# mdangschat/ctc-asr

Hardware: AMD Instinct MI355X
Metric: audio-seconds/s training throughput (DS2, 10 s utterances) (higher is better)
Workload: dtype f32 tensors / accumulate / own kernels; projection GEMMs: fp16x3 split (22 significand bits) where the layer input is bounded or, behind a ReLU cell, scaled per row / per column on the device - forward projections and their gradient GEMMs - bf16x6 split (24 bits) elsewhere; forward and backward recu

## Files before the change

ctc_asr_amd/csrc/wgrad16.hip:

```cpp
#include "common.h"

namespace {

typedef _Float16 f16x8 __attribute__((ext_vector_type(8)));
typedef unsigned int u32x4 __attribute__((ext_vector_type(4)));
union WgFrag {
    u32x4 u;
    f16x8 h;
};

constexpr int WG_THREADS = 512;
constexpr int WG_TILE = 256;
constexpr int WG_A_BYTES = (WG_TILE / 16) * 2 * 1024, WG_B_BYTES = WG_A_BYTES;
constexpr int WG_STAGE_BYTES = WG_A_BYTES + WG_B_BYTES;
constexpr size_t WG_LDS_BYTES = 2 * (size_t)WG_STAGE_BYTES;
constexpr int WG_LOADERS = 4;

struct WgArgs {
    const char *a;
    const char *b[2];
    float *out[2];
    int64_t ld[2];
    const float *inv;
    float alpha[2];
    int m, n[2], stage0[2];
    int stages, m_tiles, n_tiles[2], tiles_n[2], tiles_m;
    int parts;
    int *sync;
    long spin_limit;
};

long g_wgrad_spin_limit = 1L << 24;

__device__ __forceinline__ void wg_dma16(const char *base, unsigned lane_off, unsigned lds_base) {
    unsigned keep;
    asm volatile("s_mov_b32 %0, m0\n\ts_mov_b32 m0, %3\n\ts_nop 0\n\t"
                 "global_load_lds_dwordx4 %1, %2\n\ts_mov_b32 m0, %0"
                 : "=&s"(keep)
                 : "v"(lane_off), "s"(base), "s"(lds_base)
                 : "memory");
}

__global__ void __launch_bounds__(WG_THREADS) wgrad16_kernel(WgArgs p) {
    extern __shared__ __attribute__((aligned(16))) char smem[];
    __shared__ int gave_up;
    const int tid = threadIdx.x, lane = tid & 63;
    const int wave = __builtin_amdgcn_readfirstlane(tid >> 6);
    const int wr = wave >> 2, wc = wave & 3;
    if (p.parts > 1 &&
        __hip_atomic_load(p.sync, __ATOMIC_RELAXED, __HIP_MEMORY_SCOPE_AGENT) != 0)
        return;
    if (tid == 0) gave_up = 0;
    const int tiles_all = p.tiles_m * (p.tiles_n[0] + p.tiles_n[1]);
    const int part = blockIdx.x / tiles_all, tile_id = blockIdx.x % tiles_all;
    const int s_lo = (int)((int64_t)p.stages * part / p.parts);
    const int s_hi = (int)((int64_t)p.stages * (part + 1) / p.parts);
    int v = tile_id, which = 0;
    if (v >= p.tiles_m * p.tiles_n[0]) {
        v -= p.tiles_m * p.tiles_n[0];
        which = 1;
    }
    int tm, tn;
    {
        const int tiles_n = p.tiles_n[which], count = p.tiles_m * tiles_n;
        if (p.tiles_m % 4 == 0 && tiles_n % 4 == 0 && count % 8 == 0 &&
            (p.tiles_m * p.tiles_n[0]) % 8 == 0) {
            const int pos = (v % 8) * (count / 8) + v / 8;
            const int block = pos / 16, in_block = pos % 16, blocks_n = tiles_n / 4;
            tm = (block / blocks_n) * 4 + in_block / 4;
            tn = (block % blocks_n) * 4 + in_block % 4;
        } else {
            tm = v / tiles_n;
            tn = v % tiles_n;
        }
    }
    const int nt_total = p.n_tiles[which];
    const int mt0 = tm * (WG_TILE / 16), nt0 = tn * (WG_TILE / 16);
    const char *b_all = p.b[which] + (size_t)p.stage0[which] * nt_total * 2048;
    const unsigned lds0 = __builtin_amdgcn_readfirstlane(
        (unsigned)(uintptr_t)(__attribute__((address_space(3))) char *)smem);
    const unsigned lane16 = lane * 16;
    unsigned a_chunk[8], b_chunk[8];
#pragma unroll
    for (int c = 0; c < 8; ++c) {
        const int chunk = (wave % WG_LOADERS) * 8 + c;
        a_chunk[c] = __builtin_amdgcn_readfirstlane(
            (unsigned)(min(mt0 + (chunk >> 1), p.m_tiles - 1) * 2048 + (chunk & 1) * 1024));
        b_chunk[c] = __builtin_amdgcn_readfirstlane(
            (unsigned)(min(nt0 + (chunk >> 1), nt_total - 1) * 2048 + (chunk & 1) * 1024));
    }
    auto issue = [&](int s, unsigned buf) {
        if (wave >= WG_LOADERS) return;
        const char *a_base = p.a + (size_t)s * p.m_tiles * 2048;
        const char *b_base = b_all + (size_t)s * nt_total * 2048;
#pragma unroll
        for (int c = 0; c < 8; ++c) {
            wg_dma16(b_base + b_chunk[c], lane16, buf + WG_A_BYTES + (wave * 8 + c) * 1024);
            wg_dma16(a_base + a_chunk[c], lane16, buf + (wave * 8 + c) * 1024);
        }
    };

    f32x4 total[8][4];
#pragma unroll
    for (int i = 0; i < 8; ++i)
#pragma unroll
        for (int j = 0; j < 4; ++j) total[i][j] = (f32x4){0.f, 0.f, 0.f, 0.f};

    issue(s_lo, lds0);
    for (int s = s_lo; s < s_hi; ++s) {
        const int par = (s - s_lo) & 1;
        const char *cur = smem + par * WG_STAGE_BYTES;
        asm volatile("s_waitcnt vmcnt(0)" ::: "memory");
        __syncthreads();
        if (s + 1 < s_hi) issue(s + 1, lds0 + (par ^ 1) * WG_STAGE_BYTES);
        const char *a_rd = cur + wr * (8 * 2048) + lane * 16;
        const char *b_rd = cur + WG_A_BYTES + wc * (4 * 2048) + lane * 16;
        WgFrag x1[4], x2[4];
#pragma unroll
        for (int j = 0; j < 4; ++j) {
            x1[j].u = *reinterpret_cast<const u32x4 *>(b_rd + j * 2048);
            x2[j].u = *reinterpret_cast<const u32x4 *>(b_rd + j * 2048 + 1024);
        }
#pragma unroll
        for (int i = 0; i < 8; ++i) {
            WgFrag d1, d2;
            d1.u = *reinterpret_cast<const u32x4 *>(a_rd + i * 2048);
            d2.u = *reinterpret_cast<const u32x4 *>(a_rd + i * 2048 + 1024);
#pragma unroll
            for (int j = 0; j < 4; ++j)
                total[i][j] = __builtin_amdgcn_mfma_f32_16x16x32_f16(d1.h, x1[j].h, total[i][j], 0, 0, 0);
#pragma unroll
            for (int j = 0; j < 4; ++j)
                total[i][j] = __builtin_amdgcn_mfma_f32_16x16x32_f16(d1.h, x2[j].h, total[i][j], 0, 0, 0);
#pragma unroll
            for (int j = 0; j < 4; ++j)
                total[i][j] = __builtin_amdgcn_mfma_f32_16x16x32_f16(d2.h, x1[j].h, total[i][j], 0, 0, 0);
        }
    }

    float *out = p.out[which];
    const int64_t ld = p.ld[which];
    const float alpha = p.alpha[which];
    const int n_cols = p.n[which];
    if (p.parts == 1) {
#pragma unroll
        for (int i = 0; i < 8; ++i) {
#pragma unroll
            for (int r = 0; r < 4; ++r) {
                const int m = (mt0 + 8 * wr + i) * 16 + 4 * (lane >> 4) + r;
                if (m >= p.m) continue;
                const float scale = p.inv[m] * alpha;
                float *row = out + (int64_t)m * ld;
#pragma unroll
                for (int j = 0; j < 4; ++j) {
                    const int n = (nt0 + 4 * wc + j) * 16 + (lane & 15);
                    if (n < n_cols) row[n] += total[i][j][r] * scale;
                }
            }
        }
// ... 40 lines not shown
                const int n = (nt0 + 4 * wc + j) * 16 + (lane & 15);
                if (n < n_cols)
                    __hip_atomic_store(row + n, have[r][j] + total[i][j][r] * scale,
                                       __ATOMIC_RELAXED, __HIP_MEMORY_SCOPE_AGENT);
            }
        }
    }
    asm volatile("s_waitcnt vmcnt(0)" ::: "memory");
    __syncthreads();
    if (tid == 0)
        __hip_atomic_store(turn, part + 1 == p.parts ? 0 : part + 1, __ATOMIC_RELAXED,
                           __HIP_MEMORY_SCOPE_AGENT);
}

__global__ void __launch_bounds__(256) wgrad16_pack_kernel(const float *x, int64_t ld,
                                                           int64_t rows_total, int cols,
                                                           int64_t row0, const float *col_scale,
                                                           float scale, char *out, int col_tiles) {
    const int stage = blockIdx.x;
    const int c = blockIdx.y * 64 + (threadIdx.x & 63), kg = threadIdx.x >> 6;
    if (c >= col_tiles * 16) return;
    const float cs = (c < cols ? (col_scale ? col_scale[c] : 1.f) : 0.f) * scale;
    const int64_t r = row0 + (int64_t)stage * 32 + 8 * kg;
    unsigned pc[8];
#pragma unroll
    for (int e = 0; e < 8; ++e) {
        const int64_t row = r + e;
        float v = (c < cols && row >= 0 && row < rows_total) ? x[row * ld + c] * cs : 0.f;
        v = fminf(fmaxf(v, -60000.f), 60000.f);
        const _Float16 h1 = (_Float16)v;
        const _Float16 h2 = (_Float16)(v - (float)h1);
        pc[e] = (unsigned)__builtin_bit_cast(unsigned short, h1) |
                ((unsigned)__builtin_bit_cast(unsigned short, h2) << 16);
    }
    const u32x4 first = {(pc[0] & 0xFFFFu) | (pc[1] << 16), (pc[2] & 0xFFFFu) | (pc[3] << 16),
                         (pc[4] & 0xFFFFu) | (pc[5] << 16), (pc[6] & 0xFFFFu) | (pc[7] << 16)};
    const u32x4 second = {(pc[0] >> 16) | (pc[1] & 0xFFFF0000u), (pc[2] >> 16) | (pc[3] & 0xFFFF0000u),
                          (pc[4] >> 16) | (pc[5] & 0xFFFF0000u), (pc[6] >> 16) | (pc[7] & 0xFFFF0000u)};
    char *dst = out + (((size_t)stage * col_tiles + (c >> 4)) * 2) * 1024 + (kg * 16 + (c & 15)) * 16;
    *reinterpret_cast<u32x4 *>(dst) = first;
    *reinterpret_cast<u32x4 *>(dst + 1024) = second;
}

}

void wgrad16_set_spin_limit(long polls) { g_wgrad_spin_limit = polls > 0 ? polls : 1L << 24; }

extern "C" size_t ctcasr_wgrad16_packed_bytes(int stages, int cols) {
    return stages > 0 && cols > 0 ? (size_t)stages * ((cols + 15) / 16) * 2048 : 0;
}

extern "C" size_t ctcasr_wgrad16_sync_ints(int m, int nx, int ny) {
    const int tm = (m + WG_TILE - 1) / WG_TILE;
    return 1 + (size_t)tm * ((nx + WG_TILE - 1) / WG_TILE + (ny > 0 ? (ny + WG_TILE - 1) / WG_TILE : 0));
}

extern "C" int ctcasr_wgrad16_pack(const float *x, int64_t ld_x, int64_t rows_total, int cols,
                                   int64_t row0, int stages, const float *col_scale, float scale,
                                   void *packed, ctcasr_stream_t stream) {
    if (!x || !packed || rows_total <= 0 || cols <= 0 || ld_x < cols || stages <= 0 ||
        !(scale > 0.f))
        return CTCASR_ERR_BAD_ARGUMENT;
    const int col_tiles = (cols + 15) / 16;
    wgrad16_pack_kernel<<<dim3(stages, (col_tiles * 16 + 63) / 64), 256, 0, (hipStream_t)stream>>>(
        x, ld_x, rows_total, cols, row0, col_scale, scale, reinterpret_cast<char *>(packed),
        col_tiles);
    return ctcasr_launch_status();
}

extern "C" int ctcasr_wgrad16_gemm(const void *d_packed, int m, int stages, const float *inv_scale,
                                   const void *x_packed, int x_stage0, int nx, float x_scale,
                                   float *dw_x, int64_t ld_x, const void *y_packed, int y_stage0,
                                   int ny, float y_scale, float *dw_y, int64_t ld_y,
                                   int parts, int32_t *sync, ctcasr_stream_t stream) {
    if (!d_packed || !inv_scale || !x_packed || !dw_x || m <= 0 || stages <= 0 || nx <= 0 ||
        ld_x < nx || x_stage0 < 0 || !(x_scale > 0.f) ||
        parts < 1 || parts > stages || (parts > 1 && !sync) ||
        (y_packed && (!dw_y || ny <= 0 || ld_y < ny || y_stage0 < 0 || !(y_scale > 0.f))))
        return CTCASR_ERR_BAD_ARGUMENT;
    static bool attr_set = false;
    if (!attr_set) {
        if (hipFuncSetAttribute(reinterpret_cast<const void *>(wgrad16_kernel),
                                hipFuncAttributeMaxDynamicSharedMemorySize,
                                (int)WG_LDS_BYTES) != hipSuccess)
            return CTCASR_ERR_LAUNCH;
        attr_set = true;
    }
    WgArgs a = {};
    a.a = reinterpret_cast<const char *>(d_packed);
    a.m = m; a.stages = stages; a.inv = inv_scale;
    a.m_tiles = (m + 15) / 16;
    a.tiles_m = (m + WG_TILE - 1) / WG_TILE;
    a.b[0] = reinterpret_cast<const char *>(x_packed); a.stage0[0] = x_stage0; a.n[0] = nx;
    a.alpha[0] = 1.0f / x_scale; a.out[0] = dw_x; a.ld[0] = ld_x;
    a.n_tiles[0] = (nx + 15) / 16; a.tiles_n[0] = (nx + WG_TILE - 1) / WG_TILE;
    if (y_packed) {
        a.b[1] = reinterpret_cast<const char *>(y_packed); a.stage0[1] = y_stage0; a.n[1] = ny;
        a.alpha[1] = 1.0f / y_scale; a.out[1] = dw_y; a.ld[1] = ld_y;
        a.n_tiles[1] = (ny + 15) / 16; a.tiles_n[1] = (ny + WG_TILE - 1) / WG_TILE;
    }
    a.parts = parts; a.sync = sync; a.spin_limit = g_wgrad_spin_limit;
    const int tiles = a.tiles_m * (a.tiles_n[0] + a.tiles_n[1]) * parts;
    wgrad16_kernel<<<tiles, WG_THREADS, WG_LDS_BYTES, (hipStream_t)stream>>>(a);
    return ctcasr_launch_status();
}
```

ctc_asr_amd/hip.py:

```python

import ctypes
import functools
import os

import torch

_PKG_DIR = os.path.dirname(os.path.abspath(__file__))
LIB_PATH = os.path.join(_PKG_DIR, 'libctcasr.so')

ABI_VERSION = 7
BUILD_PROBE_WRONG_RESULTS, BUILD_NONDEFAULT_TUNING = 1, 2
RNN_DEFAULT, RNN_HALF_CHIP, RNN_WHOLE_CHIP, RNN_ONE_BARRIER = 0, 1, 2, 4
RNN_REDUCE_SCATTER = 8
RNN_F16 = 16
RNN_XCD_SPLIT = 32
RNN_STAGGER = 64
RNN_KPAIR = 128
CELL_IDS = {'rnn_relu': 0, 'rnn_tanh': 1, 'lstm': 2, 'gru': 3}
CELL_GATES = {'rnn_relu': 1, 'rnn_tanh': 1, 'lstm': 4, 'gru': 3}

_c_int, _c_i64, _c_u64 = ctypes.c_int, ctypes.c_int64, ctypes.c_uint64
_c_f, _c_p, _c_sz = ctypes.c_float, ctypes.c_void_p, ctypes.c_size_t

SIGNATURES = {
# ... 66 lines not shown
                                   _c_p]),
    'ctcasr_split_f16': (_c_int, [_c_p, _c_i64, _c_int, _c_i64, _c_f, _c_p, _c_int, _c_p, _c_i64,
                                  _c_i64, _c_p]),
    'ctcasr_colmax_scale': (_c_int, [_c_p, _c_i64, _c_int, _c_i64, _c_p, _c_p, _c_p, _c_p]),
    'ctcasr_colscale_from_max': (_c_int, [_c_p, _c_int, _c_p, _c_p, _c_p]),
    'ctcasr_split_f16_cols': (_c_int, [_c_p, _c_i64, _c_int, _c_i64, _c_p, _c_f, _c_p, _c_int, _c_p,
                                       _c_i64, _c_i64, _c_p]),
    'ctcasr_split_f16_rows': (_c_int, [_c_p, _c_i64, _c_int, _c_i64, _c_p, _c_int, _c_p, _c_i64,
                                       _c_i64, _c_p, _c_p]),
    'ctcasr_rescale_rows': (_c_int, [_c_p, _c_i64, _c_p, _c_f, _c_p, _c_i64, _c_i64, _c_int, _c_int,
                                     _c_p]),
    'ctcasr_gemm_split_nt': (_c_int, [_c_p, _c_i64, _c_p, _c_i64, _c_p, _c_i64, _c_int, _c_int, _c_int,
                                      _c_int, _c_p]),
    'ctcasr_gemm_split_tn': (_c_int, [_c_p, _c_i64, _c_p, _c_i64, _c_p, _c_i64, _c_int, _c_int, _c_int,
                                      _c_int, _c_p]),
    'ctcasr_rnn_f16_recurrence': (_c_int, [_c_int] * 7),
    'ctcasr_collective_traffic': (_c_int, [_c_int, _c_int, _c_p, _c_p, _c_i64, _c_i64, _c_p]),
    'ctcasr_wgrad16_packed_bytes': (_c_sz, [_c_int, _c_int]),
    'ctcasr_wgrad16_pack': (_c_int, [_c_p, _c_i64, _c_i64, _c_int, _c_i64, _c_int, _c_p, _c_f, _c_p,
                                     _c_p]),
    'ctcasr_wgrad16_gemm': (_c_int, [_c_p, _c_int, _c_int, _c_p, _c_p, _c_int, _c_int, _c_f, _c_p,
                                     _c_i64, _c_p, _c_int, _c_int, _c_f, _c_p, _c_i64, _c_int, _c_p,
                                     _c_p]),
    'ctcasr_wgrad16_sync_ints': (_c_sz, [_c_int, _c_int, _c_int]),
    'ctcasr_dgrad16_packed_bytes': (_c_sz, [_c_int]),
    'ctcasr_dgrad16_pack_weights': (_c_int, [_c_p, _c_i64, _c_int, _c_int, _c_f, _c_p, _c_p]),
    'ctcasr_dgrad16_supported': (_c_int, [_c_int] * 4),
    'ctcasr_dgrad16_published_offsets': (_c_int, [_c_int, _c_int, _c_int, _c_p, _c_p]),
    'ctcasr_dgrad16_blockscaled': (_c_int, [_c_p, _c_int, _c_int, _c_int, _c_p, _c_f, _c_int, _c_p,
                                            _c_i64] + [_c_int] * 5 + [_c_p]),
    'ctcasr_features_num_frames': (_c_int, [_c_int]),
    'ctcasr_features_tables_bytes': (_c_sz, []),
    'ctcasr_features_init_tables': (_c_int, [_c_p, _c_int, _c_p]),
    'ctcasr_features_workspace_bytes': (_c_sz, [_c_int, _c_int]),
    'ctcasr_features': (_c_int, [_c_p, _c_p] + [_c_int] * 5 + [_c_p, _c_p, _c_int, _c_p, _c_p,
                                 _c_sz, _c_p]),
    'ctcasr_adam_step': (_c_int, [_c_p] * 4 + [_c_i64] + [_c_f] * 4 + [_c_i64, _c_f, _c_p, _c_p]),
    'ctcasr_step_guard': (_c_int, [_c_p, _c_p, _c_int, _c_p, _c_p, _c_p, _c_p, _c_p]),
    'ctcasr_rnn_timeout_word_offset': (_c_sz, [_c_int] * 5),
    'ctcasr_absmax': (_c_int, [_c_p, _c_i64, _c_p, _c_p]),
    'ctcasr_occupy_cus': (_c_int, [_c_int, _c_int, _c_p]),
}

_lib = None

EVENTS = None
# ... 643 lines not shown

@_on_tensor_device
def wgrad16_pack(x, rows_total, row0, stages, scale, col_scale=None, out=None):
    if x.dim() != 2 or x.dtype != torch.float32 or not x.is_cuda or x.stride(1) != 1:
        raise CtcAsrError('wgrad16_pack: x must be an f32 matrix in HBM with unit column stride.')
    cols = x.shape[1]
    need = load().ctcasr_wgrad16_packed_bytes(int(stages), cols)
    if out is None:
        out = torch.empty(need, dtype=torch.uint8, device=x.device)
    elif out.dtype != torch.uint8 or out.numel() < need or not out.is_contiguous():
        raise CtcAsrError('wgrad16_pack: out must be a contiguous uint8 buffer of {} bytes.'
                          .format(need))
    _check(load().ctcasr_wgrad16_pack(
        x.data_ptr(), x.stride(0), int(rows_total), cols, int(row0), int(stages),
        _dev(col_scale, name='col_scale'), float(scale), out.data_ptr(), _stream()),
        'wgrad16_pack')
    return out


@_on_tensor_device
def wgrad16_gemm(d_packed, m, stages, inv_scale, x_packed, x_stage0, x_scale, dw_x,
                 y_packed=None, y_stage0=0, y_scale=1.0, dw_y=None, parts=1):
    parts = max(1, min(int(parts), int(stages)))
    sync = None
    if parts > 1:
        need = load().ctcasr_wgrad16_sync_ints(int(m), dw_x.shape[1], 0 if dw_y is None else dw_y.shape[1])
        sync = _WGRAD16_SYNC.get(dw_x.device.index)
        if sync is None or sync.numel() < need:
            sync = _WGRAD16_SYNC[dw_x.device.index] = torch.zeros(max(need, 4096), dtype=torch.int32,
                                                            device=dw_x.device)
    for name, t in (('dw_x', dw_x), ('dw_y', dw_y)):
        if t is not None and (t.dim() != 2 or t.dtype != torch.float32 or not t.is_cuda or
                              t.stride(1) != 1 or t.shape[0] != m):
            raise CtcAsrError('wgrad16_gemm: {} must be an f32 [m, n] view in HBM with unit '
                              'column stride.'.format(name))
    _check(load().ctcasr_wgrad16_gemm(
        d_packed.data_ptr(), int(m), int(stages), _dev(inv_scale, name='inv_scale'),
        x_packed.data_ptr(), int(x_stage0), dw_x.shape[1], float(x_scale), dw_x.data_ptr(),
        dw_x.stride(0), None if y_packed is None else y_packed.data_ptr(), int(y_stage0),
        0 if dw_y is None else dw_y.shape[1], float(y_scale),
        None if dw_y is None else dw_y.data_ptr(), 0 if dw_y is None else dw_y.stride(0),
        parts, None if sync is None else sync.data_ptr(), _stream()), 'wgrad16_gemm')


_WGRAD16_SYNC = {}


def _wgrad16_sync_of(device):
    device = torch.device(device)
    return _WGRAD16_SYNC.get(torch.cuda.current_device() if device.index is None else device.index)


def wgrad16_gave_up_waiting(device):
    sync = _wgrad16_sync_of(device)
    return bool(sync is not None and int(sync[0].item()) != 0)


def wgrad16_check(device):
    sync = _wgrad16_sync_of(device)
    if sync is not None and int(sync[0].item()) != 0:
        sync.zero_()
        torch.cuda.synchronize(sync.device)
        raise CtcAsrError('wgrad16_gemm: a part of a weight-gradient tile timed out waiting for '
                          'its turn to add; the step\'s update was not applied ({}).'.format(
                              load().ctcasr_error_string(-5).decode()))



# ... 422 lines not shown
```

ctc_asr_amd/model.py:

```python

import math
import os

import numpy as np
import torch

from ctc_asr_amd import hip, metrics, split_gemm
from ctc_asr_amd.labels import num_classes

CONV_KERNEL_SIZES = ((11, 41), (11, 21), (11, 21))
CONV_STRIDES = ((2, 2), (1, 2), (1, 2))
GATES = {'lstm': 4, 'gru': 3, 'rnn_relu': 1, 'rnn_tanh': 1}


class InfeasibleAlignmentError(ValueError):
    """Raised where ``tf.nn.ctc_loss`` raises InvalidArgumentError ("Not enough time for target
    transition sequence"), ``ignore_longer_outputs_than_inputs=False`` (``asr/model.py:259``)."""


class ModelConfig:

    def __init__(self, used_model='ds2', conv_filters=(32, 32, 96), num_units_dense=2048,
                 num_layers_rnn=4, num_units_rnn=2048, rnn_cell='rnn_relu', cudnn=True,
                 relu_cutoff=20.0, conv_dropout_rate=0.0, rnn_dropout_rate=0.0,
# ... 296 lines not shown
        self.arena = ParamArena(cfg, self.device)
        self.arena.load(params if params is not None else init_params(cfg, seed))
        self.step_count = 0
        self.overlap_wgrad = os.environ.get('CTCASR_OVERLAP_WGRAD', '1') == '1'
        self.own_conv = os.environ.get('CTCASR_OWN_CONV', '1') == '1'
        self._conv_packed = {}
        self._conv_packed16 = {}
        self.conv_f16 = os.environ.get('CTCASR_CONV_F16', '1') == '1'
        self.conv_wrw_f16 = os.environ.get('CTCASR_CONV_WRW_F16', '1') == '1'
        self.conv_fused_bwd = os.environ.get('CTCASR_CONV_FUSED_BWD', '1') == '1'
        self.side_gate_max_us = int(os.environ.get('CTCASR_SIDE_GATE_US', '300'))
        self._ticket = 0
        self.bwd_chunks = max(0, int(os.environ.get('CTCASR_BWD_CHUNKS', '0')))
        self.fwd_chunks = max(1, int(os.environ.get('CTCASR_FWD_CHUNKS', '4')))
        self.fwd_pipeline_max_batch = int(os.environ.get('CTCASR_FWD_PIPELINE_MAX_BATCH', '16'))
        self.split_gemm = os.environ.get('CTCASR_SPLIT_GEMM', '1') == '1'
        self.split_dense4 = os.environ.get('CTCASR_SPLIT_DENSE4', '1') == '1'
        self.fwd_f16 = os.environ.get('CTCASR_FWD_F16', '1') == '1'
        self.bwd_f16 = os.environ.get('CTCASR_BWD_F16', '1') == '1'
        self.split_wgrad = os.environ.get('CTCASR_SPLIT_WGRAD', '1') == '1'
        self.own_dgrad = os.environ.get('CTCASR_OWN_DGRAD', '1') == '1'
        self.own_wgrad = os.environ.get('CTCASR_OWN_WGRAD', '1') == '1'
        self.own_wgrad_parts = int(os.environ.get('CTCASR_WGRAD_PARTS', '2'))
        self.unbounded_f16 = os.environ.get('CTCASR_UNBOUNDED_F16', '1') == '1'
        self.dgrad_early = os.environ.get('CTCASR_DGRAD_EARLY', '0')
        self._dgrad_stream = None
        self.rnn_fwd_f16 = os.environ.get('CTCASR_RNN_FWD_F16', '1') == '1'
        self.rnn_bwd_f16 = os.environ.get('CTCASR_RNN_BWD_F16', '1') == '1'
        self.rnn_xcd_flag = hip.RNN_XCD_SPLIT \
            if os.environ.get('CTCASR_RNN_XCD_SPLIT', '1') == '1' else 0
        self.rnn_stagger_flag = hip.RNN_STAGGER \
            if os.environ.get('CTCASR_RNN_STAGGER', '1') == '1' else 0
        if os.environ.get('CTCASR_RNN_KPAIR', '0') == '1':
            self.rnn_stagger_flag |= hip.RNN_KPAIR
        self.rnn_kpair_wide = os.environ.get('CTCASR_RNN_KPAIR_2048', '1') == '1'
        self.rnn_fwd_pieces = os.environ.get('CTCASR_RNN_FWD_PIECES', '1') == '1'
        self._w_split, self._w_split_ready, self._w_split_bufs = {}, None, {}
        self._w_guard = None
        self._side_stream = None
        self.early_hooks = False
        self.rnn_bwd_flags = int(os.environ.get('CTCASR_RNN_BWD_FLAGS', str(hip.RNN_DEFAULT)))
        self.gpu_metrics = os.environ.get('CTCASR_GPU_METRICS', '1') == '1'
        self._rnn_ws = {}
        self.dropout_seed = int(seed) * 0x9E3779B1 + 1
        self._acts = None
        self._w_hh_t = [torch.empty((2, cfg.num_units_rnn, GATES[cfg.cell] * cfg.num_units_rnn),
# ... 644 lines not shown
                g['dense4/kernel'].zero_()
                split_gemm.wgrad16(g['dense4/kernel'], pieces.buf, inv,
                                   split_gemm.Split(dz16, split_gemm.H_B), scale, 0,
                                   x_col_inv=dz_inv)
            elif k4_split is not None:
                if dz_split is None:
                    dz_split = split_gemm.split(dz, split_gemm.B_ORDER)
                if acts['flat_split'] is None:
                    acts['flat_split'] = split_gemm.split(acts['rnn_flat'], split_gemm.A_ORDER)
                split_gemm.mm_tn_rows(g['dense4/kernel'], acts['flat_split'], dz_split, 0, rows,
                                      accumulate=False)
            else:
                torch.mm(acts['rnn_flat'].t(), dz, out=g['dense4/kernel'])
            if early:
                done('dense4')

        on_side([dz] + ([dz_split.buf] if dz_split is not None else []) +
                ([acts['flat_split'].buf] if acts['flat_split'] is not None else []),
                dense4_weight_grad, gate=True)
        if not early:
            deferred.append('dense4')

        need_dx_first = True
        rnn_rate = acts['rnn_rate']
        for i in range(cfg.num_layers_rnn - 1, -1, -1):
            name = 'rnn{}'.format(i)
            x, y = acts['layer_in'][i], acts['layer_out'][i]
            seeds = acts['drop_seeds'][i]
            if seeds[1] is not None:
                dy = hip.dropout(dy.contiguous(), rnn_rate, seeds[1])
            gh = gates * hidden
            chunks = 1
            if (side is not main and acts['rnn_len'] is None and not whole_chip_rnn and
                    persistent):
                chunks = self.bwd_chunks or 2
                if t_out < 8 * chunks:
                    chunks = 1
            dy = dy.contiguous()
            dxw = torch.empty((t_out, batch, 2, gh), dtype=torch.float32, device=dy.device)

            drec = hip.rnn_gru_drec(acts['reserves'][i], t_out, batch, hidden) if cell == 'gru' \
                else dxw
            dxw2d = dxw.view(rows, 2 * gh)
            w_ih = p[name + '/w_ih'].view(2 * gh, -1)

            w_pieces = self._weight_split(name, True, acts)
# ... 32 lines not shown

            side_tensors = [dxw] + [t.buf for t in (ds, drs, acts['in_split'][i],
                                                    acts['flat_split']) if t is not None] + \
                [t[0].buf for t in (x16, y16)
                 if t is not None and not isinstance(t, split_gemm.ColScaled)]

            def split_steps(lo, hi, ds=ds, drs=drs, dxw2d=dxw2d, drec=drec):
                for d, (a, b) in enumerate(((lo, hi), (t_out - hi, t_out - lo))):
                    rng, cols = slice(a * batch, b * batch), slice(d * gh, (d + 1) * gh)
                    hip.split_bf16(dxw2d[rng, cols], split_gemm.B_ORDER, out=ds.buf[rng, :, cols])
                    if drs is not ds:
                        hip.split_bf16(drec.view(rows, 2 * gh)[rng, cols], split_gemm.B_ORDER,
                                       out=drs.buf[rng, :, cols])

            x_packs = {}

            def partial_weight_grads_f16(lo, hi, name=name, dxw2d=dxw2d, drec=drec, x16=x16,
                                         y16=y16, x=x, y=y, colmax=None, x_packs=x_packs):
                own = (self.own_wgrad and cell != 'gru' and
                       not isinstance(x16, split_gemm.ColScaled) and
                       not isinstance(y16, split_gemm.ColScaled))
                for d, (a, b) in enumerate(((lo, hi), (t_out - hi, t_out - lo))):
                    cols = slice(d * gh, (d + 1) * gh)
                    if own:
                        n_rows = (b - a) * batch
                        stages = (n_rows + 31) // 32
                        d_rows = dxw2d[a * batch:b * batch, cols]
                        scale, inv = hip.colmax_scale(d_rows) if colmax is None else \
                            hip.colscale_from_max(colmax[d * gh:(d + 1) * gh])
                        d_pk = hip.wgrad16_pack(d_rows, n_rows, 0, stages, 1.0, col_scale=scale)
                        x_pk = x_packs.pop((a, n_rows), None)
                        if x_pk is None:
                            x_pk = hip.wgrad16_pack(x.view(rows, -1), rows, a * batch, stages,
                                                    x16[1])
                            x_packs[(a, n_rows)] = x_pk
                        y_pk = hip.wgrad16_pack(
                            y.view(rows, 2 * hidden)[:, d * hidden:(d + 1) * hidden], rows,
                            (a + (1 if d else -1)) * batch, stages, y16[1])
                        hip.wgrad16_gemm(d_pk, gh, stages, inv, x_pk, 0, x16[1],
                                         g[name + '/w_ih'][d], y_packed=y_pk, y_scale=y16[1],
                                         dw_y=g[name + '/w_hh'][d], parts=self.own_wgrad_parts)
                        continue
                    d16, inv = split_gemm.wgrad16_operand(
                        dxw2d[a * batch:b * batch, cols],
                        None if colmax is None else colmax[d * gh:(d + 1) * gh])
                    split_gemm.wgrad16(g[name + '/w_ih'][d], d16, inv, x16[0], x16[1], a * batch,
# ... 157 lines not shown
                             colmax=None if colmax is None else colmax[chunks - 1]):
                if cell != 'gru':
                    g[name + '/b_hh'].copy_(g[name + '/b_ih'])
                if chunks > 1 or use_split:
                    partial_weight_grads(0, last, colmax=colmax)
                    return
                torch.mm(dxw2d.t(), x.view(rows, -1),
                         out=g[name + '/w_ih'].view(2 * gates * hidden, -1))
                if t_out > 1:
                    gh = gates * hidden
                    torch.mm(drec[1:, :, 0, :].reshape((t_out - 1) * batch, gh).t(),
                             y[:-1, :, :hidden].reshape((t_out - 1) * batch, hidden),
                             out=g[name + '/w_hh'][0])
                    torch.mm(drec[:-1, :, 1, :].reshape((t_out - 1) * batch, gh).t(),
                             y[1:, :, hidden:].reshape((t_out - 1) * batch, hidden),
                             out=g[name + '/w_hh'][1])

            def layer_weight_grads(name=name, weight_grads=weight_grads):
                weight_grads()
                if early:
                    done(name)

            on_side(side_tensors, layer_weight_grads, gate=i > 0, beside_recurrence=i > 0)
            if not early:
                deferred.append(name)
            if dy_below is not None:
                dy = dy_below
        with torch.cuda.stream(side):
            for name in deferred:
                done(name)
            if hasattr(reduce_hook, 'flush'):
                reduce_hook.flush()

        if cfg.used_model == 'ds2':
            conv_out = acts['conv_out']
            last = conv_out[-1]
            if acts['last_time_major']:
                dact = dy.contiguous().view(last.shape)
            else:
                b_, c_, tt, ff = last.shape
                dact = dy.view(tt, b_, ff, c_).permute(1, 0, 2, 3).contiguous()
            if side is not main and any(kind is None for kind in acts['conv_own']):
                main.wait_stream(side)
            for i in range(len(cfg.conv_filters) - 1, -1, -1):
                name = 'conv{}'.format(i)
                tm = acts['last_time_major'] and i == len(cfg.conv_filters) - 1
# ... 201 lines not shown
```

include/ctcasr.h:

```cpp
#ifndef CTCASR_H_
#define CTCASR_H_

#include <stddef.h>
#include <stdint.h>

#ifdef __cplusplus
extern "C" {
#endif

#define CTCASR_ABI_VERSION 7

enum {
    CTCASR_OK = 0,
    CTCASR_ERR_BAD_ARGUMENT = -1,
    CTCASR_ERR_UNSUPPORTED = -2,
    CTCASR_ERR_WORKSPACE = -3,
    CTCASR_ERR_LAUNCH = -4,
    CTCASR_ERR_TIMEOUT = -5
};

enum {
    CTCASR_CELL_RNN_RELU = 0,
    CTCASR_CELL_RNN_TANH = 1,
    CTCASR_CELL_LSTM = 2,
// ... 174 lines not shown
int ctcasr_gemm_split_tn(const float *a, int64_t lda, const float *b, int64_t ldb, float *c,
                         int64_t ldc, int m, int n, int k, int accumulate, ctcasr_stream_t stream);

size_t ctcasr_dgrad16_packed_bytes(int n);
int ctcasr_dgrad16_published_offsets(int T, int B, int hidden, size_t *exchange,
                                     size_t *inverse_scales);
int ctcasr_dgrad16_pack_weights(const float *w_ih, int64_t ld_w, int hidden, int n, float scale,
                                void *packed, ctcasr_stream_t stream);
int ctcasr_dgrad16_supported(int cell, int T, int B, int hidden);
int ctcasr_dgrad16_blockscaled(void *workspace, int T, int B, int hidden, const void *packed,
                               float scale, int n, float *dx, int64_t ld_dx, int t_lo, int t_hi,
                               int dir_lo, int dir_hi, int accumulate, ctcasr_stream_t stream);

size_t ctcasr_wgrad16_packed_bytes(int stages, int cols);
size_t ctcasr_wgrad16_sync_ints(int m, int nx, int ny);
int ctcasr_wgrad16_pack(const float *x, int64_t ld_x, int64_t rows_total, int cols, int64_t row0,
                        int stages, const float *col_scale, float scale, void *packed,
                        ctcasr_stream_t stream);
int ctcasr_wgrad16_gemm(const void *d_packed, int m, int stages, const float *inv_scale,
                        const void *x_packed, int x_stage0, int nx, float x_scale, float *dw_x,
                        int64_t ld_x, const void *y_packed, int y_stage0, int ny, float y_scale,
                        float *dw_y, int64_t ld_y, int parts, int32_t *sync, ctcasr_stream_t stream);

int ctcasr_adam_step(float *param, const float *grad, float *m, float *v, int64_t n, float lr,
                     float beta1, float beta2, float epsilon, int64_t step, float grad_scale,
                     const int32_t *skip, ctcasr_stream_t stream);
int ctcasr_step_guard(const int32_t *ctc_status, const float *per_utterance_loss, int batch,
                      const uint32_t *timeout_word0, const uint32_t *timeout_word1,
                      const int32_t *wgrad_word, int32_t *skip, ctcasr_stream_t stream);
size_t ctcasr_rnn_timeout_word_offset(int cell, int T, int B, int H, int block);
int ctcasr_occupy_cus(int workgroups, int busy_us, ctcasr_stream_t stream);
int ctcasr_collective_traffic(int workgroups, int busy_us, float *a, const float *b,
                              int64_t scratch_floats, int64_t payload_bytes,
                              ctcasr_stream_t stream);
int ctcasr_absmax(const float *x, int64_t n, uint32_t *max_bits, ctcasr_stream_t stream);

int ctcasr_features_num_frames(int num_samples);
size_t ctcasr_features_tables_bytes(void);
int ctcasr_features_init_tables(void *tables, int sampling_rate, ctcasr_stream_t stream);
size_t ctcasr_features_workspace_bytes(int B, int max_samples);
int ctcasr_features(const int16_t *pcm, const int32_t *num_samples, int B, int max_samples,
                    int feature_type, int normalization, int drop_every_second_frame,
                    const void *tables, float *out, int out_frames, int32_t *out_len,
                    void *workspace, size_t workspace_bytes, ctcasr_stream_t stream);

#ifdef __cplusplus
// ... 4 lines not shown
```

Baseline: 6697.

## Fuse gradient packing into wgrad GEMM and share whole-layer operand packs

Adds an in-place wgrad16 kernel variant that reads the f32 gradient directly, scales it per column, splits it into fp16 hi/lo pairs and writes them to LDS inside the GEMM main loop. This removes the separate pack kernel and the packed round trip through HBM for the A operand. The model also packs each layer's x and y activations once for the whole sequence and reuses those packs across both directions, addressing them by stage and tile offsets. The cost is strided f32 global loads and split arithmetic inside the GEMM loop, more register pressure, and packs kept alive across directions.

Result: no change. 6727, median of 6 (+0.4%).

```diff
diff --git a/ctc_asr_amd/csrc/wgrad16.hip b/ctc_asr_amd/csrc/wgrad16.hip
--- a/ctc_asr_amd/csrc/wgrad16.hip
+++ b/ctc_asr_amd/csrc/wgrad16.hip
@@ -18,7 +18,12 @@
 
 struct WgArgs {
     const char *a;
+    const float *a32;
+    const float *a_scale;
+    int64_t a_ld;
+    int a_rows;
     const char *b[2];
+    int b_tiles[2], b_tile0[2];
     float *out[2];
     int64_t ld[2];
     const float *inv;
@@ -41,6 +46,24 @@
                  : "memory");
 }
 
+__device__ __forceinline__ void wg_split8(const float (&x)[8], u32x4 &first, u32x4 &second) {
+    unsigned pc[8];
+#pragma unroll
+    for (int e = 0; e < 8; ++e) {
+        float v = x[e];
+        v = fminf(fmaxf(v, -60000.f), 60000.f);
+        const _Float16 h1 = (_Float16)v;
+        const _Float16 h2 = (_Float16)(v - (float)h1);
+        pc[e] = (unsigned)__builtin_bit_cast(unsigned short, h1) |
+                ((unsigned)__builtin_bit_cast(unsigned short, h2) << 16);
+    }
+    first = (u32x4){(pc[0] & 0xFFFFu) | (pc[1] << 16), (pc[2] & 0xFFFFu) | (pc[3] << 16),
+                    (pc[4] & 0xFFFFu) | (pc[5] << 16), (pc[6] & 0xFFFFu) | (pc[7] << 16)};
+    second = (u32x4){(pc[0] >> 16) | (pc[1] & 0xFFFF0000u), (pc[2] >> 16) | (pc[3] & 0xFFFF0000u),
+                     (pc[4] >> 16) | (pc[5] & 0xFFFF0000u), (pc[6] >> 16) | (pc[7] & 0xFFFF0000u)};
+}
+
+template <bool INPLACE>
 __global__ void __launch_bounds__(WG_THREADS) wgrad16_kernel(WgArgs p) {
     extern __shared__ __attribute__((aligned(16))) char smem[];
     __shared__ int gave_up;
@@ -76,7 +99,8 @@
     }
     const int nt_total = p.n_tiles[which];
     const int mt0 = tm * (WG_TILE / 16), nt0 = tn * (WG_TILE / 16);
-    const char *b_all = p.b[which] + (size_t)p.stage0[which] * nt_total * 2048;
+    const int b_tiles = p.b_tiles[which];
+    const char *b_all = p.b[which] + ((size_t)p.stage0[which] * b_tiles + p.b_tile0[which]) * 2048;
     const unsigned lds0 = __builtin_amdgcn_readfirstlane(
         (unsigned)(uintptr_t)(__attribute__((address_space(3))) char *)smem);
     const unsigned lane16 = lane * 16;
@@ -92,13 +116,47 @@
     auto issue = [&](int s, unsigned buf) {
         if (wave >= WG_LOADERS) return;
         const char *a_base = p.a + (size_t)s * p.m_tiles * 2048;
-        const char *b_base = b_all + (size_t)s * nt_total * 2048;
+        const char *b_base = b_all + (size_t)s * b_tiles * 2048;
 #pragma unroll
         for (int c = 0; c < 8; ++c) {
             wg_dma16(b_base + b_chunk[c], lane16, buf + WG_A_BYTES + (wave * 8 + c) * 1024);
-            wg_dma16(a_base + a_chunk[c], lane16, buf + (wave * 8 + c) * 1024);
+            if (!INPLACE) wg_dma16(a_base + a_chunk[c], lane16, buf + (wave * 8 + c) * 1024);
         }
     };
+    const int a_c = tid & 255, a_kg = tid >> 8;
+    const int a_col = INPLACE ? min(mt0 * 16 + a_c, p.m - 1) : 0;
+    const float a_cs = INPLACE ? p.a_scale[a_col] : 0.f;
+    const float *a_src = INPLACE ? p.a32 + a_col : nullptr;
+    const unsigned a_dst = (a_c >> 4) * 2048 + (a_kg * 16 + (a_c & 15)) * 16;
+    float a_val[2][8];
+    auto load_a = [&](int s) {
+        const float *src = a_src + (int64_t)(s * 32 + 8 * a_kg) * p.a_ld;
+        if (s * 32 + 32 <= p.a_rows) {
+#pragma unroll
+            for (int h = 0; h < 2; ++h)
+#pragma unroll
+                for (int e = 0; e < 8; ++e) a_val[h][e] = src[(16 * h + e) * p.a_ld];
+            return;
+        }
+#pragma unroll
+        for (int h = 0; h < 2; ++h)
+#pragma unroll
+            for (int e = 0; e < 8; ++e)
+                a_val[h][e] = s * 32 + 8 * (a_kg + 2 * h) + e < p.a_rows
+                    ? src[(16 * h + e) * p.a_ld] : 0.f;
+    };
+    auto store_a = [&](char *buf) {
+#pragma unroll
+        for (int h = 0; h < 2; ++h) {
+            u32x4 first, second;
+            float v[8];
+#pragma unroll
+            for (int e = 0; e < 8; ++e) v[e] = a_val[h][e] * a_cs;
+            wg_split8(v, first, second);
+            *reinterpret_cast<u32x4 *>(buf + a_dst + h * 512) = first;
+            *reinterpret_cast<u32x4 *>(buf + a_dst + h * 512 + 1024) = second;
+        }
+    };
 
     f32x4 total[8][4];
 #pragma unroll
@@ -107,12 +165,17 @@
         for (int j = 0; j < 4; ++j) total[i][j] = (f32x4){0.f, 0.f, 0.f, 0.f};
 
     issue(s_lo, lds0);
+    if (INPLACE) {
+        load_a(s_lo);
+        store_a(smem);
+    }
     for (int s = s_lo; s < s_hi; ++s) {
         const int par = (s - s_lo) & 1;
         const char *cur = smem + par * WG_STAGE_BYTES;
         asm volatile("s_waitcnt vmcnt(0)" ::: "memory");
         __syncthreads();
         if (s + 1 < s_hi) issue(s + 1, lds0 + (par ^ 1) * WG_STAGE_BYTES);
+        if (INPLACE) load_a(min(s + 1, s_hi - 1));
         const char *a_rd = cur + wr * (8 * 2048) + lane * 16;
         const char *b_rd = cur + WG_A_BYTES + wc * (4 * 2048) + lane * 16;
         WgFrag x1[4], x2[4];
@@ -135,6 +198,10 @@
 #pragma unroll
             for (int j = 0; j < 4; ++j)
                 total[i][j] = __builtin_amdgcn_mfma_f32_16x16x32_f16(d2.h, x1[j].h, total[i][j], 0, 0, 0);
+        }
+        if (INPLACE) {
+            __builtin_amdgcn_sched_barrier(0);
+            store_a(smem + (par ^ 1) * WG_STAGE_BYTES);
         }
     }
 
@@ -221,21 +288,14 @@
     if (c >= col_tiles * 16) return;
     const float cs = (c < cols ? (col_scale ? col_scale[c] : 1.f) : 0.f) * scale;
     const int64_t r = row0 + (int64_t)stage * 32 + 8 * kg;
-    unsigned pc[8];
+    float xs[8];
 #pragma unroll
     for (int e = 0; e < 8; ++e) {
         const int64_t row = r + e;
-        float v = (c < cols && row >= 0 && row < rows_total) ? x[row * ld + c] * cs : 0.f;
-        v = fminf(fmaxf(v, -60000.f), 60000.f);
-        const _Float16 h1 = (_Float16)v;
-        const _Float16 h2 = (_Float16)(v - (float)h1);
-        pc[e] = (unsigned)__builtin_bit_cast(unsigned short, h1) |
-                ((unsigned)__builtin_bit_cast(unsigned short, h2) << 16);
-    }
-    const u32x4 first = {(pc[0] & 0xFFFFu) | (pc[1] << 16), (pc[2] & 0xFFFFu) | (pc[3] << 16),
-                         (pc[4] & 0xFFFFu) | (pc[5] << 16), (pc[6] & 0xFFFFu) | (pc[7] << 16)};
-    const u32x4 second = {(pc[0] >> 16) | (pc[1] & 0xFFFF0000u), (pc[2] >> 16) | (pc[3] & 0xFFFF0000u),
-                          (pc[4] >> 16) | (pc[5] & 0xFFFF0000u), (pc[6] >> 16) | (pc[7] & 0xFFFF0000u)};
+        xs[e] = (c < cols && row >= 0 && row < rows_total) ? x[row * ld + c] * cs : 0.f;
+    }
+    u32x4 first, second;
+    wg_split8(xs, first, second);
     char *dst = out + (((size_t)stage * col_tiles + (c >> 4)) * 2) * 1024 + (kg * 16 + (c & 15)) * 16;
     *reinterpret_cast<u32x4 *>(dst) = first;
     *reinterpret_cast<u32x4 *>(dst + 1024) = second;
@@ -267,39 +327,78 @@
     return ctcasr_launch_status();
 }
 
+namespace {
+
+bool wg_second_operand(WgArgs &a, int k, const void *packed, int stage0, int tile0, int tiles,
+                       int n, float scale, float *dw, int64_t ld) {
+    if (!packed || !dw || n <= 0 || ld < n || stage0 < 0 || tile0 < 0 || tiles < 0 ||
+        !(scale > 0.f))
+        return false;
+    const int n_tiles = (n + 15) / 16;
+    if (tiles == 0) tiles = tile0 + n_tiles;
+    if (tile0 + n_tiles > tiles) return false;
+    a.b[k] = reinterpret_cast<const char *>(packed); a.stage0[k] = stage0; a.n[k] = n;
+    a.b_tiles[k] = tiles; a.b_tile0[k] = tile0;
+    a.alpha[k] = 1.0f / scale; a.out[k] = dw; a.ld[k] = ld;
+    a.n_tiles[k] = n_tiles; a.tiles_n[k] = (n + WG_TILE - 1) / WG_TILE;
+    return true;
+}
+
+template <bool INPLACE>
+int wg_launch(WgArgs &a, int m, int stages, const float *inv_scale, int parts, int32_t *sync,
+              ctcasr_stream_t stream) {
+    static bool attr_set = false;
+    if (!attr_set) {
+        if (hipFuncSetAttribute(reinterpret_cast<const void *>(wgrad16_kernel<INPLACE>),
+                                hipFuncAttributeMaxDynamicSharedMemorySize,
+                                (int)WG_LDS_BYTES) != hipSuccess)
+            return CTCASR_ERR_LAUNCH;
+        attr_set = true;
+    }
+    a.m = m; a.stages = stages; a.inv = inv_scale;
+    a.m_tiles = (m + 15) / 16;
+    a.tiles_m = (m + WG_TILE - 1) / WG_TILE;
+    a.parts = parts; a.sync = sync; a.spin_limit = g_wgrad_spin_limit;
+    const int tiles = a.tiles_m * (a.tiles_n[0] + a.tiles_n[1]) * parts;
+    wgrad16_kernel<INPLACE><<<tiles, WG_THREADS, WG_LDS_BYTES, (hipStream_t)stream>>>(a);
+    return ctcasr_launch_status();
+}
+
+}
+
 extern "C" int ctcasr_wgrad16_gemm(const void *d_packed, int m, int stages, const float *inv_scale,
                                    const void *x_packed, int x_stage0, int nx, float x_scale,
                                    float *dw_x, int64_t ld_x, const void *y_packed, int y_stage0,
                                    int ny, float y_scale, float *dw_y, int64_t ld_y,
                                    int parts, int32_t *sync, ctcasr_stream_t stream) {
-    if (!d_packed || !inv_scale || !x_packed || !dw_x || m <= 0 || stages <= 0 || nx <= 0 ||
-        ld_x < nx || x_stage0 < 0 || !(x_scale > 0.f) ||
+    WgArgs a = {};
+    if (!d_packed || !inv_scale || m <= 0 || stages <= 0 ||
         parts < 1 || parts > stages || (parts > 1 && !sync) ||
-        (y_packed && (!dw_y || ny <= 0 || ld_y < ny || y_stage0 < 0 || !(y_scale > 0.f))))
+        !wg_second_operand(a, 0, x_packed, x_stage0, 0, 0, nx, x_scale, dw_x, ld_x) ||
+        (y_packed && !wg_second_operand(a, 1, y_packed, y_stage0, 0, 0, ny, y_scale, dw_y, ld_y)))
         return CTCASR_ERR_BAD_ARGUMENT;
-    static bool attr_set = false;
-    if (!attr_set) {
-        if (hipFuncSetAttribute(reinterpret_cast<const void *>(wgrad16_kernel),
-                                hipFuncAttributeMaxDynamicSharedMemorySize,
-                                (int)WG_LDS_BYTES) != hipSuccess)
-            return CTCASR_ERR_LAUNCH;
-        attr_set = true;
-    }
+    a.a = reinterpret_cast<const char *>(d_packed);
+    return wg_launch<false>(a, m, stages, inv_scale, parts, sync, stream);
+}
+
+extern "C" int ctcasr_wgrad16_gemm_inplace(const float *d, int64_t ld_d, int64_t rows, int m,
+                                           const float *scale, const float *inv_scale,
+                                           const void *x_packed, int x_stage0, int x_tile0,
+                                           int x_tiles, int nx, float x_scale, float *dw_x,
+                                           int64_t ld_x, const void *y_packed, int y_stage0,
+                                           int y_tile0, int y_tiles, int ny, float y_scale,
+                                           float *dw_y, int64_t ld_y, int parts, int32_t *sync,
+                                           ctcasr_stream_t stream) {
     WgArgs a = {};
-    a.a = reinterpret_cast<const char *>(d_packed);
-    a.m = m; a.stages = stages; a.inv = inv_scale;
-    a.m_tiles = (m + 15) / 16;
-    a.tiles_m = (m + WG_TILE - 1) / WG_TILE;
-    a.b[0] = reinterpret_cast<const char *>(x_packed); a.stage0[0] = x_stage0; a.n[0] = nx;
-    a.alpha[0] = 1.0f / x_scale; a.out[0] = dw_x; a.ld[0] = ld_x;
-    a.n_tiles[0] = (nx + 15) / 16; a.tiles_n[0] = (nx + WG_TILE - 1) / WG_TILE;
-    if (y_packed) {
-        a.b[1] = reinterpret_cast<const char *>(y_packed); a.stage0[1] = y_stage0; a.n[1] = ny;
-        a.alpha[1] = 1.0f / y_scale; a.out[1] = dw_y; a.ld[1] = ld_y;
-        a.n_tiles[1] = (ny + 15) / 16; a.tiles_n[1] = (ny + WG_TILE - 1) / WG_TILE;
-    }
-    a.parts = parts; a.sync = sync; a.spin_limit = g_wgrad_spin_limit;
-    const int tiles = a.tiles_m * (a.tiles_n[0] + a.tiles_n[1]) * parts;
-    wgrad16_kernel<<<tiles, WG_THREADS, WG_LDS_BYTES, (hipStream_t)stream>>>(a);
-    return ctcasr_launch_status();
-}
+    if (!d || !scale || !inv_scale || m <= 0 || ld_d < m || rows <= 0 ||
+        rows > (int64_t)INT32_MAX - 31)
+        return CTCASR_ERR_BAD_ARGUMENT;
+    const int stages = (int)((rows + 31) / 32);
+    if (parts < 1 || parts > stages || (parts > 1 && !sync) ||
+        !wg_second_operand(a, 0, x_packed, x_stage0, x_tile0, x_tiles, nx, x_scale, dw_x, ld_x) ||
+        (y_packed &&
+         !wg_second_operand(a, 1, y_packed, y_stage0, y_tile0, y_tiles, ny, y_scale, dw_y, ld_y)))
+        return CTCASR_ERR_BAD_ARGUMENT;
+    a.a32 = d; a.a_ld = ld_d; a.a_rows = (int)rows; a.a_scale = scale;
+    return wg_launch<true>(a, m, stages, inv_scale, parts, sync, stream);
+}
diff --git a/ctc_asr_amd/hip.py b/ctc_asr_amd/hip.py
--- a/ctc_asr_amd/hip.py
+++ b/ctc_asr_amd/hip.py
@@ -112,6 +112,10 @@
     'ctcasr_wgrad16_gemm': (_c_int, [_c_p, _c_int, _c_int, _c_p, _c_p, _c_int, _c_int, _c_f, _c_p,
                                      _c_i64, _c_p, _c_int, _c_int, _c_f, _c_p, _c_i64, _c_int, _c_p,
                                      _c_p]),
+    'ctcasr_wgrad16_gemm_inplace': (_c_int, [_c_p, _c_i64, _c_i64, _c_int, _c_p, _c_p,
+                                             _c_p, _c_int, _c_int, _c_int, _c_int, _c_f, _c_p, _c_i64,
+                                             _c_p, _c_int, _c_int, _c_int, _c_int, _c_f, _c_p, _c_i64,
+                                             _c_int, _c_p, _c_p]),
     'ctcasr_wgrad16_sync_ints': (_c_sz, [_c_int, _c_int, _c_int]),
     'ctcasr_dgrad16_packed_bytes': (_c_sz, [_c_int]),
     'ctcasr_dgrad16_pack_weights': (_c_int, [_c_p, _c_i64, _c_int, _c_int, _c_f, _c_p, _c_p]),
@@ -801,18 +805,7 @@
 def wgrad16_gemm(d_packed, m, stages, inv_scale, x_packed, x_stage0, x_scale, dw_x,
                  y_packed=None, y_stage0=0, y_scale=1.0, dw_y=None, parts=1):
     parts = max(1, min(int(parts), int(stages)))
-    sync = None
-    if parts > 1:
-        need = load().ctcasr_wgrad16_sync_ints(int(m), dw_x.shape[1], 0 if dw_y is None else dw_y.shape[1])
-        sync = _WGRAD16_SYNC.get(dw_x.device.index)
-        if sync is None or sync.numel() < need:
-            sync = _WGRAD16_SYNC[dw_x.device.index] = torch.zeros(max(need, 4096), dtype=torch.int32,
-                                                            device=dw_x.device)
-    for name, t in (('dw_x', dw_x), ('dw_y', dw_y)):
-        if t is not None and (t.dim() != 2 or t.dtype != torch.float32 or not t.is_cuda or
-                              t.stride(1) != 1 or t.shape[0] != m):
-            raise CtcAsrError('wgrad16_gemm: {} must be an f32 [m, n] view in HBM with unit '
-                              'column stride.'.format(name))
+    sync = _wgrad16_sync_for(m, dw_x, dw_y, parts)
     _check(load().ctcasr_wgrad16_gemm(
         d_packed.data_ptr(), int(m), int(stages), _dev(inv_scale, name='inv_scale'),
         x_packed.data_ptr(), int(x_stage0), dw_x.shape[1], float(x_scale), dw_x.data_ptr(),
@@ -822,7 +815,59 @@
         parts, None if sync is None else sync.data_ptr(), _stream()), 'wgrad16_gemm')
 
 
+@_on_tensor_device
+def wgrad16_gemm_inplace(d, scale, inv_scale, x_packed, x_stage0, x_scale, dw_x, x_tile0=0, x_tiles=0,
+                         y_packed=None, y_stage0=0, y_scale=1.0, dw_y=None, y_tile0=0, y_tiles=0,
+                         parts=1):
+    if d.dim() != 2 or d.dtype != torch.float32 or not d.is_cuda or d.stride(1) != 1 or \
+            d.shape[0] < 1:
+        raise CtcAsrError('wgrad16_gemm_inplace: d must be an f32 matrix in HBM with unit column '
+                          'stride.')
+    rows, m = d.shape
+    stages = (rows + 31) // 32
+    parts = max(1, min(int(parts), stages))
+    sync = _wgrad16_sync_for(m, dw_x, dw_y, parts)
+    for name, t in (('scale', scale), ('inv_scale', inv_scale)):
+        _expect_numel('wgrad16_gemm_inplace', name, t, m)
+    for name, pk, dw, stage0, tile0, tiles in (('x', x_packed, dw_x, x_stage0, x_tile0, x_tiles),
+                                               ('y', y_packed, dw_y, y_stage0, y_tile0, y_tiles)):
+        if pk is None:
+            continue
+        n_tiles = (dw.shape[1] + 15) // 16
+        width = int(tiles) or int(tile0) + n_tiles
+        if pk.dtype != torch.uint8 or not pk.is_contiguous() or stage0 < 0 or tile0 < 0 or \
+                tile0 + n_tiles > width or (int(stage0) + stages) * width * 2048 > pk.numel():
+            raise CtcAsrError('wgrad16_gemm_inplace: {}_packed does not hold stages [{}, {}) x '
+                              'column tiles [{}, {}) at {} tiles per stage.'.format(
+                                  name, stage0, stage0 + stages, tile0, tile0 + n_tiles, width))
+    _check(load().ctcasr_wgrad16_gemm_inplace(
+        d.data_ptr(), d.stride(0), rows, m, _dev(scale, name='scale'),
+        _dev(inv_scale, name='inv_scale'),
+        x_packed.data_ptr(), int(x_stage0), int(x_tile0), int(x_tiles), dw_x.shape[1],
+        float(x_scale), dw_x.data_ptr(), dw_x.stride(0),
+        None if y_packed is None else y_packed.data_ptr(), int(y_stage0), int(y_tile0),
+        int(y_tiles), 0 if dw_y is None else dw_y.shape[1], float(y_scale),
+        None if dw_y is None else dw_y.data_ptr(), 0 if dw_y is None else dw_y.stride(0),
+        parts, None if sync is None else sync.data_ptr(), _stream()), 'wgrad16_gemm_inplace')
+
+
 _WGRAD16_SYNC = {}
+
+
+def _wgrad16_sync_for(m, dw_x, dw_y, parts):
+    for name, t in (('dw_x', dw_x), ('dw_y', dw_y)):
+        if t is not None and (t.dim() != 2 or t.dtype != torch.float32 or not t.is_cuda or
+                              t.stride(1) != 1 or t.shape[0] != m):
+            raise CtcAsrError('wgrad16_gemm: {} must be an f32 [m, n] view in HBM with unit '
+                              'column stride.'.format(name))
+    if parts <= 1:
+        return None
+    need = load().ctcasr_wgrad16_sync_ints(int(m), dw_x.shape[1], 0 if dw_y is None else dw_y.shape[1])
+    sync = _WGRAD16_SYNC.get(dw_x.device.index)
+    if sync is None or sync.numel() < need:
+        sync = _WGRAD16_SYNC[dw_x.device.index] = torch.zeros(max(need, 4096), dtype=torch.int32,
+                                                        device=dw_x.device)
+    return sync
 
 
 def _wgrad16_sync_of(device):
diff --git a/ctc_asr_amd/model.py b/ctc_asr_amd/model.py
--- a/ctc_asr_amd/model.py
+++ b/ctc_asr_amd/model.py
@@ -342,6 +342,7 @@
         self.own_dgrad = os.environ.get('CTCASR_OWN_DGRAD', '1') == '1'
         self.own_wgrad = os.environ.get('CTCASR_OWN_WGRAD', '1') == '1'
         self.own_wgrad_parts = int(os.environ.get('CTCASR_WGRAD_PARTS', '2'))
+        self.wgrad_inplace = os.environ.get('CTCASR_WGRAD_INPLACE', '1') == '1'
         self.unbounded_f16 = os.environ.get('CTCASR_UNBOUNDED_F16', '1') == '1'
         self.dgrad_early = os.environ.get('CTCASR_DGRAD_EARLY', '0')
         self._dgrad_stream = None
@@ -1032,6 +1033,14 @@
             deferred.append('dense4')
 
         need_dx_first = True
+        layer_packs = {}
+
+        def whole_pack(t, scale):
+            key = (t.data_ptr(), scale)
+            if key not in layer_packs:
+                layer_packs[key] = hip.wgrad16_pack(t.view(rows, -1), rows, -batch,
+                                                    (t_out + 2) * batch // 32, scale)
+            return layer_packs[key]
         rnn_rate = acts['rnn_rate']
         for i in range(cfg.num_layers_rnn - 1, -1, -1):
             name = 'rnn{}'.format(i)
@@ -1110,6 +1119,36 @@
                        not isinstance(y16, split_gemm.ColScaled))
                 for d, (a, b) in enumerate(((lo, hi), (t_out - hi, t_out - lo))):
                     cols = slice(d * gh, (d + 1) * gh)
+                    if own and self.wgrad_inplace:
+                        d_rows = dxw2d[a * batch:b * batch, cols]
+                        n_rows = (b - a) * batch
+                        stages = (n_rows + 31) // 32
+                        scale, inv = hip.colmax_scale(d_rows) if colmax is None else \
+                            hip.colscale_from_max(colmax[d * gh:(d + 1) * gh])
+                        step = 1 if d else -1
+                        if batch % 32 == 0 and hidden % 16 == 0:
+                            per_step = batch // 32
+                            hip.wgrad16_gemm_inplace(
+                                d_rows, scale, inv, whole_pack(x, x16[1]), (a + 1) * per_step,
+                                x16[1], g[name + '/w_ih'][d],
+                                y_packed=whole_pack(y, y16[1]), y_stage0=(a + 1 + step) * per_step,
+                                y_scale=y16[1], dw_y=g[name + '/w_hh'][d],
+                                y_tile0=d * hidden // 16, y_tiles=2 * hidden // 16,
+                                parts=self.own_wgrad_parts)
+                            continue
+                        x_pk = x_packs.pop((a, n_rows), None)
+                        if x_pk is None:
+                            x_pk = hip.wgrad16_pack(x.view(rows, -1), rows, a * batch, stages,
+                                                    x16[1])
+                            x_packs[(a, n_rows)] = x_pk
+                        y_pk = hip.wgrad16_pack(
+                            y.view(rows, 2 * hidden)[:, d * hidden:(d + 1) * hidden], rows,
+                            (a + step) * batch, stages, y16[1])
+                        hip.wgrad16_gemm_inplace(d_rows, scale, inv, x_pk, 0, x16[1],
+                                                 g[name + '/w_ih'][d], y_packed=y_pk,
+                                                 y_scale=y16[1], dw_y=g[name + '/w_hh'][d],
+                                                 parts=self.own_wgrad_parts)
+                        continue
                     if own:
                         n_rows = (b - a) * batch
                         stages = (n_rows + 31) // 32
@@ -1313,6 +1352,11 @@
                     done(name)
 
             on_side(side_tensors, layer_weight_grads, gate=i > 0, beside_recurrence=i > 0)
+            below = acts['layer_out'][i - 1].data_ptr() if i > 0 else None
+            for key in [key for key in layer_packs if key[0] != below]:
+                pack = layer_packs.pop(key)
+                for stream in (main, side):
+                    pack.record_stream(stream)
             if not early:
                 deferred.append(name)
             if dy_below is not None:
diff --git a/include/ctcasr.h b/include/ctcasr.h
--- a/include/ctcasr.h
+++ b/include/ctcasr.h
@@ -220,6 +220,14 @@
                         int64_t ld_x, const void *y_packed, int y_stage0, int ny, float y_scale,
                         float *dw_y, int64_t ld_y, int parts, int32_t *sync, ctcasr_stream_t stream);
 
+int ctcasr_wgrad16_gemm_inplace(const float *d, int64_t ld_d, int64_t rows, int m,
+                                const float *scale, const float *inv_scale,
+                                const void *x_packed, int x_stage0, int x_tile0, int x_tiles,
+                                int nx, float x_scale, float *dw_x, int64_t ld_x,
+                                const void *y_packed, int y_stage0, int y_tile0, int y_tiles,
+                                int ny, float y_scale, float *dw_y, int64_t ld_y, int parts,
+                                int32_t *sync, ctcasr_stream_t stream);
+
 int ctcasr_adam_step(float *param, const float *grad, float *m, float *v, int64_t n, float lr,
                      float beta1, float beta2, float epsilon, int64_t step, float grad_scale,
                      const int32_t *skip, ctcasr_stream_t stream);
```
